# PositronicsLab/Moby

Measured on AMD Instinct MI355X. Metric: lcp_rows_per_sec, higher is better.
Workload: dtype f64

## Files before the change

### moby_amd/csrc/mh_lcp_wave.h

```cpp
#pragma once
#include "mh_wave.h"
#include "../../include/moby_hip.h"

namespace mh {

enum { LP_SETUP = 0, LP_GATHER, LP_LU, LP_GEMV, LP_RANDMIN, LP_VERIFY, LP_LEMKE, LP_COUNT };
__shared__ unsigned long long g_lcp_prof[LP_COUNT];
__shared__ int g_lcp_prof_on;
#ifdef MH_PROFILE_BUILD
MH_DEV void lds_add(unsigned long long* p, unsigned long long v) {
  if (lane_id() == 0) (void)__hip_atomic_fetch_add(p, v, __ATOMIC_RELAXED, __HIP_MEMORY_SCOPE_WAVEFRONT);
}
MH_DEV unsigned long long lp_tick() { return g_lcp_prof_on ? __builtin_amdgcn_s_memtime() : 0ull; }
MH_DEV void lp_tock(int ph, unsigned long long t0) { if (g_lcp_prof_on) { const unsigned long long d = __builtin_amdgcn_s_memtime() - t0; lds_add(&g_lcp_prof[ph], d); } }
#else
MH_DEV unsigned long long lp_tick() { return 0ull; }
MH_DEV void lp_tock(int, unsigned long long) {}
#endif

struct Trace {
  int32_t* buf; int cap; int len;
  MH_DEV void push(int32_t v) { if (buf && len < cap && lane_id() == 0) buf[len] = v; len++; }
};

#define MH_DBL_EPS 2.220446049250313e-16
#define MH_NEAR_ZERO 1.4901161193847656e-08
#define MH_SFMIN 2.2250738585072014e-308

struct DenseLds {
  const double* M; int n;
  MH_DEV double at_row(int c) const { const int l = lane_id(); return (l < n) ? M[l + n * c] : 0.0; }
  MH_DEV double diag() const { const int l = lane_id(); return (l < n) ? M[l + n * l] : 0.0; }
  MH_DEV double offdiag_max() const {
    const int lane = lane_id();
    double m = 0.0;
    if (lane < n)
      for (int c = 0; c < n; c++) {
        const double a = fabs(M[lane + n * c]);
        if (c != lane && a > m) m = a;
      }
    return wave_max(m);
  }
};

template <class MatT>
MH_DEV double mat_at(const MatT& M, int c, double lam) {
  const double m = M.at_row(c);
  return (lane_id() == c) ? m + lam : m;
}

MH_DEV int lu_solve_wave(int k, double* A, double& b)
{
  const int lane = lane_id();
  for (int j = 0; j < k; j++) {
    const bool mine = (lane >= j) && (lane < k);
    double a = mine ? fabs(A[lane + k * j]) : -1.0;
    double amax; int jp;
    argmax_first(a, mine, amax, jp);
    if (!(amax != 0.0)) return j + 1;
    if (jp != j) {
      if (lane < k) { double t0 = A[j + k * lane], t1 = A[jp + k * lane]; A[j + k * lane] = t1; A[jp + k * lane] = t0; }
      double bj = read_lane(b, j), bjp = read_lane(b, jp);
      if (lane == j) b = bjp; else if (lane == jp) b = bj;
      wave_sync();
    }
    if (j < k - 1) {
      const double piv = A[j + k * j];
      if (lane > j && lane < k) {
        double l = A[lane + k * j];
        if (fabs(piv) >= MH_SFMIN) { const double r = 1.0 / piv; l = l * r; } else l = l / piv;
        A[lane + k * j] = l;
        for (int c0 = j + 1; c0 < k; c0 += 8) {
          double a[8], u[8];
#pragma unroll
          for (int t = 0; t < 8; t++) {
            const int c = (c0 + t < k) ? c0 + t : k - 1;
            a[t] = A[lane + k * c]; u[t] = A[j + k * c];
          }
#pragma unroll
          for (int t = 0; t < 8; t++)
            if (c0 + t < k) A[lane + k * (c0 + t)] = a[t] - l * u[t];
        }
      }
      wave_sync();
    }
  }
  for (int kk = 0; kk < k; kk++) {
    const double bk = read_lane(b, kk);
    if (lane > kk && lane < k) b = b - bk * A[lane + k * kk];
  }
  for (int kk = k - 1; kk >= 0; kk--) {
    if (lane == kk) b = b / A[kk + k * kk];
    const double bk = read_lane(b, kk);
    if (lane < kk) b = b - bk * A[lane + k * kk];
  }
  return 0;
}

MH_DEV int lu_solve_wave_hbm(int k, double* A, double& b)
{
  constexpr int PB = 8;
  const int lane = lane_id();
  const bool valid = lane < k;
  int prow = lane;
  for (int j0 = 0; j0 < k; j0 += PB) {
    const int nb = (k - j0 < PB) ? k - j0 : PB;
    double p[PB];
#pragma unroll
    for (int c = 0; c < PB; c++) p[c] = (valid && c < nb) ? A[prow + k * (j0 + c)] : 0.0;
#pragma unroll
    for (int jj = 0; jj < PB; jj++) {
      if (jj < nb) {
        const int j = j0 + jj;
        const bool mine = (lane >= j) && valid;
        double amax; int jp;
        argmax_first(mine ? fabs(p[jj]) : -1.0, mine, amax, jp);
        if (!(amax != 0.0)) return j + 1;
        if (jp != j) {
#pragma unroll
          for (int c = 0; c < PB; c++) { const double vj = read_lane(p[c], j), vp = read_lane(p[c], jp); if (lane == j) p[c] = vp; else if (lane == jp) p[c] = vj; }
          { const double vj = read_lane(b, j), vp = read_lane(b, jp); if (lane == j) b = vp; else if (lane == jp) b = vj; }
          { const int rj = read_lane(prow, j), rp = read_lane(prow, jp); if (lane == j) prow = rp; else if (lane == jp) prow = rj; }
        }
        if (j < k - 1) {
          const double piv = read_lane(p[jj], j);
          const bool below = (lane > j) && valid;
          if (below) { double l = p[jj]; if (fabs(piv) >= MH_SFMIN) { const double r = 1.0 / piv; l = l * r; } else l = l / piv; p[jj] = l; }
#pragma unroll
          for (int c = 0; c < PB; c++) if (c > jj && c < nb) { const double u = read_lane(p[c], j); if (below) p[c] = p[c] - p[jj] * u; }
        }
      }
    }
#pragma unroll
    for (int c = 0; c < PB; c++) if (valid && c < nb) A[prow + k * (j0 + c)] = p[c];
    for (int cb = j0 + nb; cb < k; cb += PB) {
      double a[PB];
#pragma unroll
      for (int u = 0; u < PB; u++) a[u] = (valid && cb + u < k) ? A[prow + k * (cb + u)] : 0.0;
#pragma unroll
      for (int u = 0; u < PB; u++) {
#pragma unroll
        for (int s2 = 0; s2 < PB; s2++) if (s2 < nb) { const double us = read_lane(a[u], j0 + s2); if (lane > j0 + s2 && valid) a[u] = a[u] - p[s2] * us; }
      }
#pragma unroll
      for (int u = 0; u < PB; u++) if (valid && cb + u < k) A[prow + k * (cb + u)] = a[u];
    }
  }
  wave_sync();
  for (int kb = 0; kb < k; kb += PB) {
    double l[PB];
#pragma unroll
    for (int u = 0; u < PB; u++) l[u] = (valid && kb + u < k) ? A[prow + k * (kb + u)] : 0.0;
#pragma unroll
    for (int u = 0; u < PB; u++) if (kb + u < k) { const double bk = read_lane(b, kb + u); if (lane > kb + u && valid) b = b - bk * l[u]; }
  }
  for (int ke = k; ke > 0; ke -= PB) {
    const int kb = (ke - PB > 0) ? ke - PB : 0;
    double uu[PB];
#pragma unroll
    for (int u = 0; u < PB; u++) uu[u] = (valid && kb + u < ke) ? A[prow + k * (kb + u)] : 1.0;
#pragma unroll
    for (int u = PB - 1; u >= 0; u--) if (kb + u < ke) {
      const int kk = kb + u;
      if (lane == kk) b = b / uu[u];
      const double bk = read_lane(b, kk);
      if (lane < kk) b = b - bk * uu[u];
    }
  }
  return 0;
}

MH_DEV int rand_min_wave(double v, uint64_t mask, double tol, WaveRand& rng, double& val, bool& tie)
{
  const int lane = lane_id();
  const bool in = (mask >> lane) & 1ull;
  double vmin; int imin;
  if (popc(mask) <= 4) {
    uint64_t m = mask;
    imin = ctz(m); m &= m - 1;
    vmin = read_lane(v, imin);
    while (m) { const int i = ctz(m); m &= m - 1; const double x = read_lane(v, i); if (x < vmin) { vmin = x; imin = i; } }
  } else argmin_first(v, in, vmin, imin);
  const uint64_t qm = ballot(in && lane != imin && v < vmin + tol);
  const int cnt = 1 + popc(qm);
  tie = tie || cnt > 1;
  const int rv = rng.next();
  const int r = (cnt == 1) ? 0 : rv % cnt;
  const int chosen = (r == 0) ? imin : nth_set_bit(qm, r - 1);
  val = read_lane(v, chosen);
  return chosen;
}

MH_DEV double norm_reg(double offmax, double dii, bool valid, double lam) {
  double d = valid ? fabs(dii + lam) : 0.0;
  double m = wave_max(d);
  return (m > offmax) ? m : offmax;
}

struct LuScratch { double* small; int ka; double* big; };

template <int K>
MH_DEV int lu_small(const double* A, double& b)
{
  double a[K][K], x[K];
#pragma unroll
  for (int c = 0; c < K; c++)
#pragma unroll
    for (int r = 0; r < K; r++) a[r][c] = A[r + K * c];
#pragma unroll
  for (int r = 0; r < K; r++) x[r] = read_lane(b, r);
#pragma unroll
  for (int j = 0; j < K; j++) {
    int jp = j; double amax = fabs(a[j][j]);
#pragma unroll
    for (int i = j + 1; i < K; i++) { const double v = fabs(a[i][j]); if (v > amax) { amax = v; jp = i; } }
    jp = uni(jp);
    if (ballot(!(amax != 0.0)) != 0ull) return j + 1;
#pragma unroll
    for (int i = j + 1; i < K; i++)
      if (jp == i) {
#pragma unroll
        for (int c = 0; c < K; c++) { const double t = a[j][c]; a[j][c] = a[i][c]; a[i][c] = t; }
        const double t = x[j]; x[j] = x[i]; x[i] = t;
      }
    if (j < K - 1) {
      const double piv = a[j][j];
      const bool big = fabs(piv) >= MH_SFMIN;
      const double r = 1.0 / piv;
#pragma unroll
      for (int i = j + 1; i < K; i++) {
        const double l = big ? a[i][j] * r : a[i][j] / piv;
        a[i][j] = l;
#pragma unroll
        for (int c = j + 1; c < K; c++) a[i][c] = a[i][c] - l * a[j][c];
      }
    }
  }
#pragma unroll
  for (int kk = 0; kk < K; kk++)
#pragma unroll
    for (int i = kk + 1; i < K; i++) x[i] = x[i] - x[kk] * a[i][kk];
#pragma unroll
  for (int kk = K - 1; kk >= 0; kk--) {
    x[kk] = x[kk] / a[kk][kk];
#pragma unroll
    for (int i = 0; i < kk; i++) x[i] = x[i] - x[kk] * a[i][kk];
  }
  const int lane = lane_id();
  double out = 0.0;
#pragma unroll
  for (int r = 0; r < K; r++) out = (lane == r) ? x[r] : out;
  b = out;
  return 0;
}

#ifndef MH_COLCACHE
#define MH_COLCACHE 4
#endif
template <bool REGLU, class MatT>
MH_DEV int gather_and_solve(const MatT& M, double lam, uint64_t nbmask, int k, bool is_nb, int pos, double qi, double* A, double& b,
                            double (&colv)[MH_COLCACHE])
{
  const int lane = lane_id();
  unsigned long long t0 = lp_tick();
  if (k == 1) {
    const int j = ctz(nbmask);
    const double v = mat_at(M, j, lam);
    colv[0] = v;
    const double a00 = read_lane(v, j);
    const double rhs = read_lane(-qi, j);
    lp_tock(LP_GATHER, t0);
    if (!(fabs(a00) != 0.0)) return 1;
    b = (lane == 0) ? rhs / a00 : 0.0;
    return 0;
  }
  wave_sync();
  uint64_t m = nbmask;
#pragma unroll
  for (int c = 0; c < MH_COLCACHE; c++) {
    if (c < k) {
      const int j = ctz(m); m &= m - 1;
      const double v = mat_at(M, j, lam);
      colv[c] = v;
      if (is_nb) A[pos + k * c] = v;
    }
  }
  for (int c = MH_COLCACHE; c < k; c++) {
    const int j = ctz(m); m &= m - 1;
    const double v = mat_at(M, j, lam);
    if (is_nb) A[pos + k * c] = v;
  }
  b = push_to(-qi, is_nb ? pos : k + popc(~nbmask & lanes_below(lane)));
  wave_sync();
  lp_tock(LP_GATHER, t0);
  t0 = lp_tick();
  int info;
  if (REGLU && k == 2) info = lu_small<2>(A, b);
  else if (REGLU && k == 3) info = lu_small<3>(A, b);
#ifndef MH_NO_LU4
  else if (REGLU && k == 4) info = lu_small<4>(A, b);
#endif
  else info = REGLU ? lu_solve_wave(k, A, b) : lu_solve_wave_hbm(k, A, b);
  lp_tock(LP_LU, t0);
  return info;
}

template <class MatT>
MH_DEV bool lcp_fast_wave(int n, const MatT& M, double lam, LuScratch S,
                          double qi, double& zi, int& zsize, double zero_tol,
                          double nrm_lam, WaveRand& rng, unsigned& pivots, Trace& tr)
{
  const int lane = lane_id();
  const bool valid = lane < n;
  const uint64_t vmask = lanes_below(n);
  if (zero_tol < 0.0) zero_tol = (double)n * nrm_lam * MH_DBL_EPS;
  uint64_t nbmask;
  if (zsize == n) {
    nbmask = ballot(valid && !(fabs(zi) < zero_tol));
  } else {
    double qmin; int minw;
    argmin_first(qi, valid, qmin, minw);
    if (qmin > -zero_tol) { zi = 0.0; zsize = n; pivots = 0; return true; }
    nbmask = bit(minw);
  }
  const unsigned MAX_PIV = 2u * (unsigned)n;
  for (pivots = 0; pivots < MAX_PIV; pivots++) {
    const int k = popc(nbmask);
    const bool is_nb = (nbmask >> lane) & 1ull;
    const bool is_b = valid && !is_nb;
    const int pos = popc(nbmask & lanes_below(lane));
    double b = 0.0;
    double colv[MH_COLCACHE];
    if (k > 0) {
      int info;
      if (k <= S.ka) info = gather_and_solve<true>(M, lam, nbmask, k, is_nb, pos, qi, S.small, b, colv);
      else info = gather_and_solve<false>(M, lam, nbmask, k, is_nb, pos, qi, S.big, b, colv);
      if (info != 0) return false;
    }
    unsigned long long tg = lp_tick();
    double w = 0.0;
    {
      uint64_t m = nbmask;
#pragma unroll
      for (int c = 0; c < MH_COLCACHE; c++) {
        if (c < k) {
          m &= m - 1;
          const double t = read_lane(b, c);
          if (is_b) w = w + t * colv[c];
        }
      }
      for (int c = MH_COLCACHE; c < k; c++) {
        const int j = ctz(m); m &= m - 1;
        const double t = read_lane(b, c);
        const double v = mat_at(M, j, lam);
        if (is_b) w = w + t * v;
      }
      w = w + qi;
    }
    const double zv = __shfl(b, pos);
    lp_tock(LP_GEMV, tg);
    tg = lp_tick();
    const uint64_t bmask = vmask & ~nbmask;
    double wsel = 0.0; int minw = -1;
    bool tie = false;
    if (bmask != 0ull) {
      if (ballot(is_b && !(w > -zero_tol)) == 0ull) (void)rng.next();
      else minw = rand_min_wave(w, bmask, zero_tol, rng, wsel, tie);
    }
    double zsel = 0.0; int minz = -1;
    if (k > 0) {
      if (ballot(is_nb && !(zv >= -zero_tol)) == 0ull) (void)rng.next();
      else minz = rand_min_wave(zv, nbmask, zero_tol, rng, zsel, tie);
    }
    lp_tock(LP_RANDMIN, tg);
    if (minw < 0 || wsel > -zero_tol) {
      if (minz >= 0 && zsel < -zero_tol) {
        nbmask &= ~bit(minz);
        tr.push(-(int32_t)(minz + 1));
      } else {
        zi = is_nb ? zv : 0.0;
        zsize = n;
        return true;
      }
    } else {
      const uint64_t nb_new = nbmask | bit(minw);
      tr.push((int32_t)(minw + 1));
      nbmask = nb_new;
      if (minz >= 0 && zsel < -zero_tol) {
        const int posz = popc((nb_new & ~bit(minw)) & lanes_below(minz));
        const int idx2 = nth_set_bit(nb_new, posz);
        nbmask &= ~bit(idx2);
        tr.push(-(int32_t)(idx2 + 1));
#ifndef MH_NO_REPEAT_SKIP
        if (idx2 == minw && !tie) {
          const unsigned rest = MAX_PIV - (pivots + 1u);
          rng.skip(2u * rest);
          if (tr.buf && tr.len < tr.cap) for (unsigned r = 0; r < rest; r++) { tr.push((int32_t)(minw + 1)); tr.push(-(int32_t)(idx2 + 1)); }
          else tr.len += (int)(2u * rest);
          pivots = MAX_PIV;
          return false;
        }
#endif
      }
    }
  }
  return false;
}

template <class MatT>
MH_DEV bool verify_wave(int n, const MatT& M, double lam, double qi, double zi, double ZERO_TOL, bool strict)
{
  const int lane = lane_id();
  const bool valid = lane < n;
  const double nT = -ZERO_TOL;
  if (ballot(valid && zi != zi) != 0ull) { const double mz = min_element_value(zi, valid); if (!(strict ? (mz > nT) : (mz >= nT))) return false; }
  else if (ballot(valid && !(strict ? (zi > nT) : (zi >= nT))) != 0ull) return false;
  double w = 0.0;
  uint64_t nz = ballot(valid && zi != 0.0);
  while (nz) {
    const int c = ctz(nz); nz &= nz - 1;
    const double t = read_lane(zi, c);
    const double m = mat_at(M, c, lam);
    if (valid) w = w + t * m;
  }
  w = w + qi;
  const double zw = zi * w;
  if (ballot(valid && (w != w || zw != zw)) != 0ull) {
    const double mw = min_element_value(w, valid);
    if (!(strict ? (mw > nT) : (mw >= nT))) return false;
    const double mn = min_element_value(zw, valid), mx = max_element_value(zw, valid);
    return (strict ? (mn > nT) : (mn >= nT)) && mx < ZERO_TOL;
  }
  if (ballot(valid && !(strict ? (w > nT) : (w >= nT))) != 0ull) return false;
  if (ballot(valid && !(strict ? (zw > nT) : (zw >= nT))) != 0ull) return false;
  return ballot(valid && !(zw < ZERO_TOL)) == 0ull;
}

template <bool HBM, class MatT>
MH_DEV int lemke_gather_and_solve(int n, const MatT& M, double lam, int bv, int t, const double* art, double* A, double& d)
{
  const int lane = lane_id();
  const bool valid = lane < n;
  wave_sync();
  for (int p = 0; p < n; p++) {
    const int id = read_lane(bv, p);
    double a;
    if (id == t) a = valid ? art[lane] : 0.0;
    else if (id >= n) a = (lane == id - n) ? -1.0 : 0.0;
    else a = mat_at(M, id, lam);
    if (valid) A[lane + n * p] = a;
  }
  wave_sync();
  return HBM ? lu_solve_wave_hbm(n, A, d) : lu_solve_wave(n, A, d);
}

template <class MatT>
MH_DEV bool lcp_lemke_wave(int n, const MatT& M, double lam, LuScratch S, double* art,
                           double qi, double& zi, int& zsize, double piv_tol, double zero_tol,
                           double nrm_lam, WaveRand& rng, unsigned& pivots, Trace& tr)
{
  const int lane = lane_id();
  const bool valid = lane < n;
  const double INF = __longlong_as_double(0x7ff0000000000000ll);
  const unsigned MAXITER = (50u * (unsigned)n < 1000u) ? 50u * (unsigned)n : 1000u;
  pivots = 0;
  zi = 0.0;
  const int z0size = zsize;
  if (zero_tol <= 0.0) zero_tol = MH_DBL_EPS * nrm_lam * (double)n;
  const double qmin = wave_min(valid ? qi : INF);
  if (qmin > -zero_tol) { zsize = n; return true; }
  zsize = 2 * n;
  const int t = 2 * n;
  if (z0size != n) for (int i = 0; i < n; i++) (void)rng.next();
  int bv = n + lane;
  double x = valid ? qi : 0.0;
  if (ballot(valid && x < 0.0) == 0ull) { zsize = n; return true; }
  const double PIV_TOL = (piv_tol > 0.0) ? piv_tol : MH_DBL_EPS * (double)n * ((nrm_lam > 1.0) ? nrm_lam : 1.0);
  double xmin; int lvindex;
  argmin_first(x, valid, xmin, lvindex);
  const double tval = -xmin;
  int leaving = n + lvindex;
  int entering = t;
  double u = (valid && x < 0.0) ? 1.0 : 0.0;
  wave_sync();
  if (valid) art[lane] = u;
  u = u * tval;
  x = x + u;
  if (lane == lvindex) { x = tval; bv = t; }
  wave_sync();
  for (pivots = 0; pivots < MAXITER; pivots++) {
    if (leaving == t) {
      wave_sync();
      if (valid) art[lane] = 0.0;
      wave_sync();
      if (valid && bv < n) art[bv] = x;
      wave_sync();
      zi = valid ? art[lane] : 0.0;
      zsize = n;
      return true;
    }
    double be;
    if (leaving < n) { entering = n + leaving; be = (lane == leaving) ? -1.0 : 0.0; }
    else { entering = leaving - n; be = valid ? mat_at(M, entering, lam) : 0.0; }
    double d = be;
    {
      int info;
      if (n <= S.ka) info = lemke_gather_and_solve<false>(n, M, lam, bv, t, art, S.small, d);
      else info = lemke_gather_and_solve<true>(n, M, lam, bv, t, art, S.big, d);
      if (info != 0) return false;
    }
    const uint64_t jm = ballot(valid && d > PIV_TOL);
    if (jm == 0ull) return false;
    const bool inj = (jm >> lane) & 1ull;
    const double rat = inj ? (x + zero_tol) / d : INF;
    { const double r0 = read_lane(rat, ctz(jm)); if (r0 != r0) { zsize = n; return false; } }
    const double theta = wave_min(rat);
    const uint64_t keep = ballot(inj && (x / d <= theta));
    if (keep == 0ull) { zsize = n; return false; }
    const uint64_t tm = ballot(valid && bv == t);
    lvindex = (keep & tm) ? ctz(tm) : ctz(keep);
    leaving = read_lane(bv, lvindex);
    const double ratio = read_lane(x, lvindex) / read_lane(d, lvindex);
    d = d * ratio;
    x = x - d;
    if (lane == lvindex) { x = ratio; bv = entering; }
    tr.push((int32_t)entering + 1); tr.push((int32_t)leaving + 1);
  }
  zsize = n;
  return false;
}


struct LcpParams { int kind; int min_exp; unsigned step_exp; int max_exp; double piv_tol; double zero_tol; };

struct Pow10Table { double v[64]; };

template <class MatT>
MH_DEV bool lcp_solve_wave(const LcpParams& P, const Pow10Table& p10, int n, const MatT& M, LuScratch A, double* art,
                           double nrm0, double dii, double qi, double& zi, int& zsize,
                           WaveRand& rng, unsigned& pivots, Trace& tr)
{
  const bool valid = lane_id() < n;
  const bool reg = (P.kind == MH_LCP_FAST_REG) || (P.kind == MH_LCP_LEMKE_REG);
  const bool fast = (P.kind == MH_LCP_FAST) || (P.kind == MH_LCP_FAST_REG);
  const double ZERO_TOL = (P.zero_tol > 0.0) ? P.zero_tol : (double)n * nrm0 * MH_NEAR_ZERO;
  unsigned total = 0;
  double offmax = 0.0;
  int rf = P.min_exp;
  for (int attempt = 0; ; attempt++) {
    double lam = 0.0, nrm = nrm0;
    if (attempt > 0) {
      if (!reg || !(rf < P.max_exp)) break;
      if (attempt == 1) offmax = M.offdiag_max();
      lam = p10.v[rf + 32];
      nrm = norm_reg(offmax, dii, valid, lam);
    }
    if (reg) tr.push(0x40000000 | attempt);
    unsigned long long tl = lp_tick();
    const bool ok = fast ? lcp_fast_wave(n, M, lam, A, qi, zi, zsize, P.zero_tol, nrm, rng, pivots, tr)
                         : lcp_lemke_wave(n, M, lam, A, art, qi, zi, zsize, P.piv_tol, P.zero_tol, nrm, rng, pivots, tr);
    if (!fast) lp_tock(LP_LEMKE, tl);
    if (!reg) return ok;
    tl = lp_tick();
    const bool good = ok && verify_wave(n, M, lam, qi, zi, ZERO_TOL, attempt > 0);
    lp_tock(LP_VERIFY, tl);
    if (attempt == 0) { if (good) return true; total += pivots; }
    else { total += pivots; if (good) { pivots = total; return true; } rf += (int)P.step_exp; }
  }
  pivots = total;
  return false;
}

}
```

Baseline: 2.442 billion.

## Solve small LCP pivot systems entirely in registers via lane reads

Adds a small_iteration path for basis sizes up to 4 that gathers matrix columns into registers and builds the LU system with cross-lane reads instead of staging it through LDS scratch with wave syncs. The gemv and z extraction for this path run on per-lane register values. It also special-cases k==0 and k==1 pivot selection and uses a mask instead of modulo when the tie count is a power of two. The cost is more cross-lane reads per element and extra code paths. Any divergence from the old RNG consumption order would change pivot traces.

```diff
diff --git a/moby_amd/csrc/mh_lcp_wave.h b/moby_amd/csrc/mh_lcp_wave.h
--- a/moby_amd/csrc/mh_lcp_wave.h
+++ b/moby_amd/csrc/mh_lcp_wave.h
@@ -173,8 +173,8 @@
 MH_DEV int rand_min_wave(double v, uint64_t mask, double tol, WaveRand& rng, double& val, bool& tie)
 {
   const int lane = lane_id();
+  double vmin; int imin;
   const bool in = (mask >> lane) & 1ull;
-  double vmin; int imin;
   if (popc(mask) <= 4) {
     uint64_t m = mask;
     imin = ctz(m); m &= m - 1;
@@ -185,7 +185,7 @@
   const int cnt = 1 + popc(qm);
   tie = tie || cnt > 1;
   const int rv = rng.next();
-  const int r = (cnt == 1) ? 0 : rv % cnt;
+  const int r = ((cnt & (cnt - 1)) == 0) ? (rv & (cnt - 1)) : rv % cnt;
   const int chosen = (r == 0) ? imin : nth_set_bit(qm, r - 1);
   val = read_lane(v, chosen);
   return chosen;
@@ -200,15 +200,15 @@
 struct LuScratch { double* small; int ka; double* big; };
 
 template <int K>
-MH_DEV int lu_small(const double* A, double& b)
+MH_DEV int lu_small(const int (&jr)[4], const double (&col)[4], double nq, double (&xo)[4])
 {
   double a[K][K], x[K];
 #pragma unroll
   for (int c = 0; c < K; c++)
 #pragma unroll
-    for (int r = 0; r < K; r++) a[r][c] = A[r + K * c];
-#pragma unroll
-  for (int r = 0; r < K; r++) x[r] = read_lane(b, r);
+    for (int r = 0; r < K; r++) a[r][c] = read_lane(col[c], jr[r]);
+#pragma unroll
+  for (int r = 0; r < K; r++) x[r] = read_lane(nq, jr[r]);
 #pragma unroll
   for (int j = 0; j < K; j++) {
     int jp = j; double amax = fabs(a[j][j]);
@@ -246,34 +246,72 @@
 #pragma unroll
     for (int i = 0; i < kk; i++) x[i] = x[i] - x[kk] * a[i][kk];
   }
-  const int lane = lane_id();
-  double out = 0.0;
-#pragma unroll
-  for (int r = 0; r < K; r++) out = (lane == r) ? x[r] : out;
-  b = out;
+#pragma unroll
+  for (int r = 0; r < K; r++) xo[r] = x[r];
   return 0;
 }
 
 #ifndef MH_COLCACHE
 #define MH_COLCACHE 4
 #endif
+#ifndef MH_NO_LU4
+#define MH_REGLU_MAX 4
+#else
+#define MH_REGLU_MAX 3
+#endif
+
+template <class MatT>
+MH_DEV int small_iteration(const MatT& M, double lam, uint64_t nbmask, int k, double qi, double& w, double& zv)
+{
+  unsigned long long t0 = lp_tick();
+  int jr[4]; double col[4];
+  uint64_t m = nbmask;
+#pragma unroll
+  for (int c = 0; c < 4; c++) {
+    jr[c] = ctz(m);
+    if (c < k) { m &= m - 1; col[c] = mat_at(M, jr[c], lam); }
+  }
+  lp_tock(LP_GATHER, t0);
+  t0 = lp_tick();
+  double x[4];
+  int info = 0;
+  if (k == 1) {
+    const double a00 = read_lane(col[0], jr[0]);
+    const double rhs = read_lane(-qi, jr[0]);
+    if (!(fabs(a00) != 0.0)) return 1;
+    x[0] = uni(rhs / a00);
+  }
+  else if (k == 2) info = lu_small<2>(jr, col, -qi, x);
+#ifndef MH_NO_LU4
+  else if (k == 4) info = lu_small<4>(jr, col, -qi, x);
+#endif
+  else info = lu_small<3>(jr, col, -qi, x);
+  lp_tock(LP_LU, t0);
+  if (info != 0) return info;
+  t0 = lp_tick();
+  w = 0.0;
+#pragma unroll
+  for (int c = 0; c < MH_REGLU_MAX; c++) if (c < k) w = w + x[c] * col[c];
+  w = w + qi;
+  zv = x[0];
+  if (k > 1) {
+    const int pos = popc(nbmask & lanes_below(lane_id()));
+#pragma unroll
+    for (int r = 1; r < MH_REGLU_MAX; r++) if (r < k) zv = (pos == r) ? x[r] : zv;
+  }
+  lp_tock(LP_GEMV, t0);
+  return 0;
+}
+
 template <bool REGLU, class MatT>
-MH_DEV int gather_and_solve(const MatT& M, double lam, uint64_t nbmask, int k, bool is_nb, int pos, double qi, double* A, double& b,
-                            double (&colv)[MH_COLCACHE])
-{
-  const int lane = lane_id();
+MH_DEV int general_iteration(const MatT& M, double lam, uint64_t nbmask, int k, bool is_nb, bool is_b, double qi, double* A,
+                             double& w, double& zv)
+{
+  const int lane = lane_id();
+  const int pos = popc(nbmask & lanes_below(lane));
   unsigned long long t0 = lp_tick();
-  if (k == 1) {
-    const int j = ctz(nbmask);
-    const double v = mat_at(M, j, lam);
-    colv[0] = v;
-    const double a00 = read_lane(v, j);
-    const double rhs = read_lane(-qi, j);
-    lp_tock(LP_GATHER, t0);
-    if (!(fabs(a00) != 0.0)) return 1;
-    b = (lane == 0) ? rhs / a00 : 0.0;
-    return 0;
-  }
+  double b;
+  double colv[MH_COLCACHE];
   wave_sync();
   uint64_t m = nbmask;
 #pragma unroll
@@ -294,15 +332,30 @@
   wave_sync();
   lp_tock(LP_GATHER, t0);
   t0 = lp_tick();
-  int info;
-  if (REGLU && k == 2) info = lu_small<2>(A, b);
-  else if (REGLU && k == 3) info = lu_small<3>(A, b);
-#ifndef MH_NO_LU4
-  else if (REGLU && k == 4) info = lu_small<4>(A, b);
-#endif
-  else info = REGLU ? lu_solve_wave(k, A, b) : lu_solve_wave_hbm(k, A, b);
+  const int info = REGLU ? lu_solve_wave(k, A, b) : lu_solve_wave_hbm(k, A, b);
   lp_tock(LP_LU, t0);
-  return info;
+  if (info != 0) return info;
+  t0 = lp_tick();
+  w = 0.0;
+  m = nbmask;
+#pragma unroll
+  for (int c = 0; c < MH_COLCACHE; c++) {
+    if (c < k) {
+      m &= m - 1;
+      const double t = read_lane(b, c);
+      if (is_b) w = w + t * colv[c];
+    }
+  }
+  for (int c = MH_COLCACHE; c < k; c++) {
+    const int j = ctz(m); m &= m - 1;
+    const double t = read_lane(b, c);
+    const double v = mat_at(M, j, lam);
+    if (is_b) w = w + t * v;
+  }
+  w = w + qi;
+  zv = __shfl(b, pos);
+  lp_tock(LP_GEMV, t0);
+  return 0;
 }
 
 template <class MatT>
@@ -326,40 +379,29 @@
   const unsigned MAX_PIV = 2u * (unsigned)n;
   for (pivots = 0; pivots < MAX_PIV; pivots++) {
     const int k = popc(nbmask);
+    if (k == 0) {
+      const unsigned long long tg = lp_tick();
+      const double w = 0.0 + qi;
+      double wsel = 0.0; int minw = -1; bool tie = false;
+      if (ballot(valid && !(w > -zero_tol)) == 0ull) (void)rng.next();
+      else minw = rand_min_wave(w, vmask, zero_tol, rng, wsel, tie);
+      lp_tock(LP_RANDMIN, tg);
+      if (minw < 0 || wsel > -zero_tol) { zi = 0.0; zsize = n; return true; }
+      nbmask = bit(minw);
+      tr.push((int32_t)(minw + 1));
+      continue;
+    }
     const bool is_nb = (nbmask >> lane) & 1ull;
     const bool is_b = valid && !is_nb;
-    const int pos = popc(nbmask & lanes_below(lane));
-    double b = 0.0;
-    double colv[MH_COLCACHE];
-    if (k > 0) {
+    double w, zv;
+    {
       int info;
-      if (k <= S.ka) info = gather_and_solve<true>(M, lam, nbmask, k, is_nb, pos, qi, S.small, b, colv);
-      else info = gather_and_solve<false>(M, lam, nbmask, k, is_nb, pos, qi, S.big, b, colv);
+      if (k == 1 || (k <= MH_REGLU_MAX && k <= S.ka)) info = small_iteration(M, lam, nbmask, k, qi, w, zv);
+      else if (k <= S.ka) info = general_iteration<true>(M, lam, nbmask, k, is_nb, is_b, qi, S.small, w, zv);
+      else info = general_iteration<false>(M, lam, nbmask, k, is_nb, is_b, qi, S.big, w, zv);
       if (info != 0) return false;
     }
-    unsigned long long tg = lp_tick();
-    double w = 0.0;
-    {
-      uint64_t m = nbmask;
-#pragma unroll
-      for (int c = 0; c < MH_COLCACHE; c++) {
-        if (c < k) {
-          m &= m - 1;
-          const double t = read_lane(b, c);
-          if (is_b) w = w + t * colv[c];
-        }
-      }
-      for (int c = MH_COLCACHE; c < k; c++) {
-        const int j = ctz(m); m &= m - 1;
-        const double t = read_lane(b, c);
-        const double v = mat_at(M, j, lam);
-        if (is_b) w = w + t * v;
-      }
-      w = w + qi;
-    }
-    const double zv = __shfl(b, pos);
-    lp_tock(LP_GEMV, tg);
-    tg = lp_tick();
+    const unsigned long long tg = lp_tick();
     const uint64_t bmask = vmask & ~nbmask;
     double wsel = 0.0; int minw = -1;
     bool tie = false;
@@ -368,10 +410,14 @@
       else minw = rand_min_wave(w, bmask, zero_tol, rng, wsel, tie);
     }
     double zsel = 0.0; int minz = -1;
-    if (k > 0) {
-      if (ballot(is_nb && !(zv >= -zero_tol)) == 0ull) (void)rng.next();
-      else minz = rand_min_wave(zv, nbmask, zero_tol, rng, zsel, tie);
-    }
+    if (k == 1) {
+      (void)rng.next();
+      const int j = ctz(nbmask);
+      const double z = read_lane(zv, j);
+      if (!(z >= -zero_tol)) { minz = j; zsel = z; }
+    }
+    else if (ballot(is_nb && !(zv >= -zero_tol)) == 0ull) (void)rng.next();
+    else minz = rand_min_wave(zv, nbmask, zero_tol, rng, zsel, tie);
     lp_tock(LP_RANDMIN, tg);
     if (minw < 0 || wsel > -zero_tol) {
       if (minz >= 0 && zsel < -zero_tol) {
```

Result: no change. 2.456 billion (median of 6 runs) (+0.6%).
